# Balaji-Kesavan/DistributedDataparallel

Hardware: AMD Instinct MI355X
Metric: images/sec (whole node) ResNet-50 DDP at 1/2/4/8 MI355X; scaling efficiency (higher is better)
Workload: dtype bf16; 1 GPU; model=resnet50, global_batch=256, per_gpu_batch=256, micro_batch=256, image_size=224, parallelism=dp1, impl=xddp, backend=rccl, norm=xddp, optimizer=SGD(lr=0.1, momentum=0.9, wd=0.0001) fp32 master weights, recipe=default, miopen_implicit_gemm=default, optimizer_schedule=after backward, channels_last=True, comm_dtype=none, gradient_as_bucket_view=True

## Files before the change

distributeddataparallel_amd/csrc/kernels/conv_gemm.hip:

```cpp
#include <c10/hip/HIPStream.h>
#include <torch/extension.h>

#include "common.h"
#include "kernels/dev_utils.h"

namespace xddp {
namespace kernels {

namespace {

typedef __bf16 bf16x8 __attribute__((ext_vector_type(8)));
using dev::f32x4;
using dev::u32x4;

constexpr int kBK = 64;
constexpr bool NTSTORE = true;

__device__ __forceinline__ int swz(int row, int chunk) { return row * 128 + 16 * (chunk ^ ((row >> 1) & 7)); }

__device__ __forceinline__ void lds_barrier() { asm volatile("s_waitcnt lgkmcnt(0)\n\ts_barrier" ::: "memory"); }

__device__ __forceinline__ float bf16_round(float v) { return __uint_as_float(dev::pack_bf16x2(v, 0.f) << 16); }

typedef short v4s __attribute__((ext_vector_type(4)));

__device__ __forceinline__ v4s lds_tr16(const uint8_t* p) {
  return __builtin_amdgcn_ds_read_tr16_b64_v4i16((__attribute__((address_space(3))) v4s*)(p));
}

struct EpiBN {
  const uint16_t* add;
  const uint16_t* y;
  const uint8_t* bits;
  const float* mean;
  float* part;
  const float* ss;
  int add_h, add_w;
};

struct ProOut {
  uint16_t* out;
  uint8_t* bits;
  const float* rss;
  int64_t* nbt1;
  int64_t* nbt2;
};

struct RowMap {
  int OH, OW, IH, IW, stride;
  template <bool STRIDED>
  __device__ __forceinline__ int64_t in_row(int m) const {
    if (!STRIDED) return m;
    const int hw = OH * OW;
    const int n = m / hw, r = m - n * hw;
    const int oh = r / OW, ow = r - oh * OW;
    return ((int64_t)n * IH + oh * stride) * IW + (int64_t)ow * stride;
  }
};

template <int BM, int BN, int WM, int WN, int PRO, bool STATS, bool STRIDED, bool BT = false, bool EPI = false,
          int OCC = 4>
__global__ __launch_bounds__(64 * WM * WN, OCC) void conv1x1_gemm_kernel(
    const uint16_t* __restrict__ X, const uint16_t* __restrict__ Wt, uint16_t* __restrict__ Y, int64_t M, int N,
    int K, RowMap rm, const float* __restrict__ pro_ss, float* __restrict__ part, int mtiles, int ntiles,
    int groups, const uint16_t* __restrict__ X2, EpiBN epi, ProOut po) {
  static_assert(PRO < 4 || (!STRIDED && !BT && !EPI), "the block-output prologue is a stride-1 forward");
  constexpr int NT = 64 * WM * WN, RSTEP = NT / 8;
  constexpr int AR = BM / RSTEP, BR = BN / RSTEP;
  constexpr int WTM = BM / WM, WTN = BN / WN;
  constexpr int TM = WTM / 16, TN = WTN / 16;
  constexpr int SBT = BN * 2 + 32;
  constexpr int ABYTES = BM * 128, BBYTES = BT ? 64 * SBT : BN * 128, BUF = ABYTES + BBYTES;
  extern __shared__ __attribute__((aligned(16))) uint8_t smem[];

  const int tid = threadIdx.x, lane = tid & 63, wid = tid >> 6, wm = wid / WN, wn = wid % WN;
  const int wg = dev::xcd_remap(blockIdx.x, gridDim.x);
  const int nt = wg % ntiles, g = wg / ntiles;
  if (g >= groups) return;
  const int n0 = nt * BN;
  const int lc = tid & 7, lr = tid >> 3;
  const int nk = K / kBK;

  constexpr int CPR = BN / 8;
  static_assert(NT % CPR == 0, "readout mapping needs a fixed chunk column per thread");
  const int cc = tid % CPR;
  float st_s[8], st_ss[8];
#pragma unroll
  for (int e = 0; e < 8; ++e) st_s[e] = st_ss[e] = 0.f;
  constexpr int SPR = BN / 2, SRS = NT / SPR;
  static_assert(SPR <= 64 && 64 % SPR == 0 && BM % SRS == 0, "stats pass mapping");
  const int sp = tid % SPR;
  float sn = 0.f, sk[2] = {0.f, 0.f}, ssum[2] = {0.f, 0.f}, ssq[2] = {0.f, 0.f};

  const uint16_t* wrow[BR];
  constexpr int BCH = BN / 8;
  static_assert(!BT || 64 * BCH == NT * BR, "BT staging must cover the B tile exactly");
#pragma unroll
  for (int i = 0; i < BR; ++i) {
    if (BT) {
      const int q = tid + NT * i, row = q / BCH, c = q % BCH;
      wrow[i] = Wt + (int64_t)row * N + n0 + c * 8;
    } else {
      wrow[i] = Wt + (int64_t)(n0 + lr + RSTEP * i) * K + lc * 8;
    }
  }

  u32x4 sa[AR], sb[BR], sa2[PRO >= 2 ? AR : 1];
  float* pro_lds = reinterpret_cast<float*>(smem + 2 * BUF);
  constexpr int NCOEF = PRO == 3 ? 5 : PRO == 2 ? 3 : PRO == 5 ? 4 : PRO ? 2 : 0;
// ... 437 lines not shown
  const float dm = n > 0.f ? s1 / n : 0.f;
  const float mean = K + dm;
  const float m2 = fmaxf(s2 - s1 * dm, 0.f);
  const float Mf = M > 0 ? (float)M : n;
  const float var = Mf > 0.f ? fmaxf(m2 / Mf, 0.f) : 0.f;
  const float inv = rsqrtf(var + eps);
  mean_out[c] = mean;
  invstd_out[c] = inv;
  scale[c] = gm * inv;
  shift[c] = bb - mean * gm * inv;
  if (running_mean) {
    const float unbiased = Mf > 1.f ? var * Mf / (Mf - 1.f) : var;
    dev::Elem<W, float>::st(running_mean, c, (1.f - mom) * rm + mom * mean);
    dev::Elem<W, float>::st(running_var, c, (1.f - mom) * rv + mom * unbiased);
  }
}



template <int TN, int TK, bool STRIDED, int PRO>
__global__ __launch_bounds__(256, 2) void conv1x1_wgrad_kernel(const uint16_t* __restrict__ dY,
                                                                const uint16_t* __restrict__ X,
                                                                float* __restrict__ ws, int M, int N, int K,
                                                                RowMap rm, int ntiles, int ktiles, int mchunk,
                                                                const uint16_t* __restrict__ Y2,
                                                                const float* __restrict__ coef) {
  constexpr int BM = 64;
  constexpr int SA = TN * 2 + 32, SB = TK * 2 + 32;
  constexpr int ABYTES = BM * SA, BUF = ABYTES + BM * SB;
  constexpr int CA = TN / 8, CB = TK / 8;
  constexpr int LA = BM * CA / 256, LB = BM * CB / 256;
  constexpr int WTN = TN / 2, WTK = TK / 2, FN = WTN / 16, FK = WTK / 16;
  extern __shared__ __attribute__((aligned(16))) uint8_t smem[];

  const int tid = threadIdx.x, lane = tid & 63, wid = tid >> 6, wn = wid >> 1, wk = wid & 1;
  const int tiles = ntiles * ktiles;
  const int bid = dev::xcd_remap(blockIdx.x, gridDim.x);
  const int sidx = bid / tiles, tile = bid % tiles;
  const int n0 = (tile % ntiles) * TN, k0 = (tile / ntiles) * TK;
  const int m_begin = sidx * mchunk, m_end = min(M, m_begin + mchunk);

  u32x4 sa[2][LA], sb[2][LB], sa2[2][PRO ? LA : 1];
  float pa[8], pb[8], pc[8], pms[8], pmt[8];
  if (PRO) {
    const int c = tid % CA;
    dev::Vec8<float>::ld(coef + n0 + c * 8, pa);
    dev::Vec8<float>::ld(coef + N + n0 + c * 8, pb);
    dev::Vec8<float>::ld(coef + 2 * N + n0 + c * 8, pc);
    if (PRO == 3) {
      dev::Vec8<float>::ld(coef + 3 * N + n0 + c * 8, pms);
      dev::Vec8<float>::ld(coef + 4 * N + n0 + c * 8, pmt);
    }
  }
  auto load = [&](int slot, int m) {
#pragma unroll
    for (int i = 0; i < LA; ++i) {
      const int q = tid + 256 * i, row = q / CA, c = q - (q / CA) * CA;
      const int64_t off = (int64_t)min(m + row, M - 1) * N + n0 + c * 8;
      sa[slot][i] = *reinterpret_cast<const u32x4*>(dY + off);
      if (PRO) sa2[slot][i] = *reinterpret_cast<const u32x4*>(Y2 + off);
    }
#pragma unroll
    for (int i = 0; i < LB; ++i) {
      const int q = tid + 256 * i, row = q / CB, c = q - (q / CB) * CB;
      sb[slot][i] = *reinterpret_cast<const u32x4*>(X + rm.in_row<STRIDED>(min(m + row, M - 1)) * K + k0 + c * 8);
    }
  };
  auto store = [&](int buf, int slot, int m) {
    uint8_t* A = smem + buf * BUF;
    uint8_t* B = A + ABYTES;
#pragma unroll
    for (int i = 0; i < LA; ++i) {
      const int q = tid + 256 * i, row = q / CA, c = q - (q / CA) * CA;
      u32x4 t = sa[slot][i];
      if (PRO) {
#pragma unroll
        for (int h = 0; h < 4; ++h) {
          float g0 = __uint_as_float(sa[slot][i][h] << 16), g1 = __uint_as_float(sa[slot][i][h] & 0xffff0000u);
          const float x0 = __uint_as_float(sa2[slot][i][h] << 16), x1 = __uint_as_float(sa2[slot][i][h] & 0xffff0000u);
          if (PRO == 3) {
            g0 = fmaf(x0, pms[2 * h], pmt[2 * h]) > 0.f ? g0 : 0.f;
            g1 = fmaf(x1, pms[2 * h + 1], pmt[2 * h + 1]) > 0.f ? g1 : 0.f;
          }
          t[h] = dev::pack_bf16x2(fmaf(pa[2 * h], g0, fmaf(pb[2 * h], x0, pc[2 * h])),
                                  fmaf(pa[2 * h + 1], g1, fmaf(pb[2 * h + 1], x1, pc[2 * h + 1])));
        }
      }
      *reinterpret_cast<u32x4*>(A + row * SA + c * 16) = m + row < m_end ? t : u32x4{0, 0, 0, 0};
    }
#pragma unroll
    for (int i = 0; i < LB; ++i) {
      const int q = tid + 256 * i, row = q / CB, c = q - (q / CB) * CB;
      *reinterpret_cast<u32x4*>(B + row * SB + c * 16) = m + row < m_end ? sb[slot][i] : u32x4{0, 0, 0, 0};
    }
  };

  f32x4 acc[FN][FK];
#pragma unroll
  for (int i = 0; i < FN; ++i)
#pragma unroll
    for (int j = 0; j < FK; ++j) acc[i][j] = f32x4{0.f, 0.f, 0.f, 0.f};

  const int g = lane >> 4, q4 = (lane & 15) >> 2, p4 = lane & 3;
  auto compute = [&](int cur) {
    const uint8_t* A = smem + cur * BUF;
    const uint8_t* B = A + ABYTES;
#pragma unroll
    for (int s2 = 0; s2 < 2; ++s2) {
      const int r0 = s2 * 32 + 8 * g + q4;
      bf16x8 a[FN], b[FK];
#pragma unroll
      for (int i = 0; i < FN; ++i) {
        const int col = wn * WTN + i * 16 + 4 * p4;
        const v4s lo = lds_tr16(A + r0 * SA + col * 2), hi = lds_tr16(A + (r0 + 4) * SA + col * 2);
        const v4s v8[2] = {lo, hi};
        a[i] = __builtin_bit_cast(bf16x8, v8);
      }
#pragma unroll
      for (int j = 0; j < FK; ++j) {
        const int col = wk * WTK + j * 16 + 4 * p4;
        const v4s lo = lds_tr16(B + r0 * SB + col * 2), hi = lds_tr16(B + (r0 + 4) * SB + col * 2);
        const v4s v8[2] = {lo, hi};
        b[j] = __builtin_bit_cast(bf16x8, v8);
      }
#pragma unroll
      for (int i = 0; i < FN; ++i)
#pragma unroll
        for (int j = 0; j < FK; ++j) acc[i][j] = __builtin_amdgcn_mfma_f32_16x16x32_bf16(a[i], b[j], acc[i][j], 0, 0, 0);
    }
  };
  if (m_begin < m_end) {
    load(0, m_begin);
    load(1, m_begin + BM);
    store(0, 0, m_begin);
    lds_barrier();
    for (int m = m_begin; m < m_end; m += 2 * BM) {
      load(0, m + 2 * BM);
      compute(0);
      store(1, 1, m + BM);
      lds_barrier();
      if (m + BM >= m_end) break;
      load(1, m + 3 * BM);
      compute(1);
      store(0, 0, m + 2 * BM);
      lds_barrier();
    }
    asm volatile("s_waitcnt vmcnt(0)" ::: "memory");
  }
  float* out = ws + (int64_t)sidx * N * K;
#pragma unroll
  for (int i = 0; i < FN; ++i)
#pragma unroll
    for (int j = 0; j < FK; ++j)
#pragma unroll
      for (int r = 0; r < 4; ++r) {
        const int n = n0 + wn * WTN + i * 16 + (lane >> 4) * 4 + r;
        const int k = k0 + wk * WTK + j * 16 + (lane & 15);
        out[(int64_t)n * K + k] = acc[i][j][r];
      }
}

template <int N, int K, int PRO>
__global__ __launch_bounds__(256, 1) void conv1x1_bwd_fused_kernel(
    const uint16_t* __restrict__ G, const uint16_t* __restrict__ Y2, const float* __restrict__ coef,
    const uint16_t* __restrict__ X, const uint16_t* __restrict__ Wg, uint16_t* __restrict__ dX, float* __restrict__ ws,
    int M, int mchunk) {
  constexpr int BM = 64;
  constexpr int SA = N * 2 + 32, SB = K * 2 + 32, SW = K * 2 + 32;
  constexpr int ABYTES = BM * SA, BUF = ABYTES + BM * SB;
  constexpr int CA = N / 8, CB = K / 8;
  constexpr int LA = BM * CA / 256, LB = BM * CB / 256;
  constexpr int WTN = N / 2, WTK = K / 2, FN = WTN / 16, FK = WTK / 16;
  constexpr int KW = K / 4, KF = KW / 16;
  static_assert(256 % CA == 0 && LA >= 1 && LB >= 1 && KF >= 1, "fused 1x1 backward tile");
  extern __shared__ __attribute__((aligned(16))) uint8_t smem[];
  uint8_t* Wl = smem + 2 * BUF;

  const int tid = threadIdx.x, lane = tid & 63, wid = tid >> 6, wn = wid >> 1, wk = wid & 1;
  const int bid = dev::xcd_remap(blockIdx.x, gridDim.x);
  const int m_begin = bid * mchunk, m_end = min(M, m_begin + mchunk);

  for (int q = tid; q < N * CB; q += 256) {
    const int n = q / CB, c = q % CB;
    *reinterpret_cast<u32x4*>(Wl + n * SW + c * 16) = *reinterpret_cast<const u32x4*>(Wg + (int64_t)n * K + c * 8);
  }
  float pa[8], pb[8], pc[8], pms[8], pmt[8];
  {
    const int c = tid % CA;
    dev::Vec8<float>::ld(coef + c * 8, pa);
    dev::Vec8<float>::ld(coef + N + c * 8, pb);
    dev::Vec8<float>::ld(coef + 2 * N + c * 8, pc);
    if (PRO == 3) {
      dev::Vec8<float>::ld(coef + 3 * N + c * 8, pms);
      dev::Vec8<float>::ld(coef + 4 * N + c * 8, pmt);
    }
  }
  u32x4 sa[LA], sa2[LA], sb[LB];
  auto load = [&](int m) {
#pragma unroll
    for (int i = 0; i < LA; ++i) {
// ... 299 lines not shown
    epi = EpiBN{reinterpret_cast<const uint16_t*>(epi_add->data_ptr()), reinterpret_cast<const uint16_t*>(epi_y->data_ptr()),
                epi_bits->data_ptr<uint8_t>(), epi_mean->data_ptr<float>(), part.data_ptr<float>(), nullptr,
                epi_add_stride == 2 ? (int)OH : 0, epi_add_stride == 2 ? (int)OW : 0};
  else if (epi_form2)
    epi = EpiBN{nullptr, reinterpret_cast<const uint16_t*>(epi_y->data_ptr()), nullptr, epi_mean->data_ptr<float>(),
                part.data_ptr<float>(), epi_ss->data_ptr<float>(), 0, 0};
  RowMap rm{(int)OH, (int)OW, (int)IH, (int)IW, (int)stride};
  const dim3 grid(groups * ntiles);
  const size_t bbytes = w_t ? (size_t)64 * (BN * 2 + 32) : (size_t)BN * 128;
  const size_t lds = 2 * ((size_t)BM * 128 + bbytes) + (pro ? (pro == 5 ? 4 : ncoef) * K * sizeof(float) : 0) +
                     (epi_on ? 3 * (size_t)BN * sizeof(float) : 0);
  const auto* x2p = pro >= 4 ? reinterpret_cast<const uint16_t*>(pro_res->data_ptr())
                   : pro >= 2 ? reinterpret_cast<const uint16_t*>(prologue_y->data_ptr()) : nullptr;
  const ProOut po{def(pro_out) ? reinterpret_cast<uint16_t*>(pro_out->data_ptr()) : nullptr,
                  def(pro_bits) ? pro_bits->data_ptr<uint8_t>() : nullptr,
                  has_rss ? pro_res_ss->data_ptr<float>() : nullptr,
                  def(pro_nbt) ? pro_nbt->data_ptr<int64_t>() : nullptr,
                  def(pro_res_nbt) ? pro_res_nbt->data_ptr<int64_t>() : nullptr};
  const auto* xp = reinterpret_cast<const uint16_t*>(x.data_ptr());
  const auto* wp = reinterpret_cast<const uint16_t*>(wc.data_ptr());
  auto* yp = reinterpret_cast<uint16_t*>(y.data_ptr());
  const float* pss = pro ? prologue_ss->data_ptr<float>() : nullptr;
  float* pp = stats ? part.data_ptr<float>() : nullptr;
#define XDDP_LG(BN_, WM_, WN_, OCC_)                                                                            \
  launch_gemm<128, BN_, WM_, WN_, OCC_>(pro, stats, w_t, grid, lds, stream, xp, wp, yp, M, (int)N, (int)K, rm, pss, pp, \
                                        mtiles, ntiles, groups, x2p, epi, po)
  if (pro >= 4) {
    auto go = [&](auto kern) {
      ensure_dyn_lds((const void*)kern, lds);
      hipLaunchKernelGGL(kern, grid, dim3(512), lds, stream, xp, wp, yp, M, (int)N, (int)K, rm, pss, pp, mtiles, ntiles,
                         groups, x2p, epi, po);
    };
#define XDDP_P45(BM_, BN_, WM_, WN_)                                                                     \
    if (pro == 5) { if (stats) go(conv1x1_gemm_kernel<BM_, BN_, WM_, WN_, 5, true, false, false, false, 4>);    \
                    else go(conv1x1_gemm_kernel<BM_, BN_, WM_, WN_, 5, false, false, false, false, 4>); }   \
    else { if (stats) go(conv1x1_gemm_kernel<BM_, BN_, WM_, WN_, 4, true, false, false, false, 4>);             \
           else go(conv1x1_gemm_kernel<BM_, BN_, WM_, WN_, 4, false, false, false, false, 4>); }
    if (BN == 128) { XDDP_P45(64, 128, 2, 4) } else { XDDP_P45(128, 64, 8, 1) }
#undef XDDP_P45
    XDDP_HIP_CHECK(hipGetLastError());
  } else if (bm64) {
    auto kern = pro == 2 ? conv1x1_gemm_kernel<64, 128, 2, 4, 2, false, false, true, true, 4>
                         : conv1x1_gemm_kernel<64, 128, 2, 4, 0, false, false, true, true, 4>;
    hipLaunchKernelGGL(kern, grid, dim3(512), lds, stream, xp, wp, yp, M, (int)N, (int)K, rm, pss, pp, mtiles, ntiles,
                       groups, x2p, epi, po);
    XDDP_HIP_CHECK(hipGetLastError());
  } else if (BN == 128) { if (kocc == 2) XDDP_LG(128, 4, 2, 2); else XDDP_LG(128, 4, 2, 4); }
  else { if (kocc == 2) XDDP_LG(64, 8, 1, 2); else XDDP_LG(64, 8, 1, 4); }
#undef XDDP_LG
  return {y, part};
}


at::Tensor conv1x1_wgrad(const at::Tensor& dy, const at::Tensor& x, int64_t stride, const at::Tensor& w_like,
                         const c10::optional<at::Tensor>& prologue_y, const c10::optional<at::Tensor>& coef) {
  const auto wdtype = w_like.scalar_type();
  const bool has_y2 = prologue_y.has_value() && prologue_y->defined();
  const int pro = has_y2 ? (coef.has_value() && coef->defined() && coef->numel() == 5 * dy.size(1) ? 3 : 2) : 0;
  TORCH_CHECK(dy.is_cuda() && x.is_cuda() && dy.scalar_type() == at::kBFloat16 && x.scalar_type() == at::kBFloat16,
              "conv1x1_wgrad: bf16 GPU tensors expected");
  TORCH_CHECK(dy.dim() == 4 && x.dim() == 4 && dy.is_contiguous(at::MemoryFormat::ChannelsLast) &&
                  x.is_contiguous(at::MemoryFormat::ChannelsLast), "conv1x1_wgrad: channels_last 4-D tensors expected");
  const int64_t B = x.size(0), K = x.size(1), IH = x.size(2), IW = x.size(3), N = dy.size(1);
  const int64_t OH = (IH - 1) / stride + 1, OW = (IW - 1) / stride + 1;
  TORCH_CHECK(dy.size(0) == B && dy.size(2) == OH && dy.size(3) == OW, "conv1x1_wgrad: dy/x shape mismatch");
  TORCH_CHECK(N % 64 == 0 && K % 64 == 0, "conv1x1_wgrad: channel counts must be multiples of 64");
  const int64_t M = B * OH * OW;
  TORCH_CHECK(M > 0 && M < (int64_t(1) << 31), "conv1x1_wgrad: bad M");
  if (pro)
    TORCH_CHECK(prologue_y->sizes() == dy.sizes() && prologue_y->scalar_type() == at::kBFloat16 &&
                    prologue_y->is_contiguous(at::MemoryFormat::ChannelsLast) && stride == 1 && coef.has_value() &&
                    coef->defined() && coef->scalar_type() == at::kFloat && coef->numel() == (pro == 3 ? 5 : 3) * N &&
                    coef->is_contiguous(),
                "conv1x1_wgrad: prologue_y must match dy (bf16 channels_last, stride 1) with float coef [3|5, N]");
  const auto* y2p = pro ? reinterpret_cast<const uint16_t*>(prologue_y->data_ptr()) : nullptr;
  const float* cfp = pro ? coef->data_ptr<float>() : nullptr;
  const int TN = N % 128 == 0 ? 128 : 64, TK = K % 128 == 0 ? 128 : 64;
  const int ntiles = (int)(N / TN), ktiles = (int)(K / TK), tiles = ntiles * ktiles;
  const int64_t steps = (M + 63) / 64;
  int S = (int)std::max<int64_t>(1, std::min<int64_t>(steps, (int64_t)num_cus() * 2 / tiles));
  const int64_t mchunk = ((steps + S - 1) / S) * 64;
  S = (int)((M + mchunk - 1) / mchunk);
  auto ws = at::empty({S, N, K}, dy.options().dtype(at::kFloat));
  auto dw = at::empty({N, K, 1, 1}, dy.options().dtype(wdtype));
  auto stream = c10::hip::getCurrentHIPStream(dy.device().index()).stream();
  RowMap rm{(int)OH, (int)OW, (int)IH, (int)IW, (int)stride};
  const size_t lds = 2 * (size_t)64 * ((TN * 2 + 32) + (TK * 2 + 32));
  auto go = [&](auto kern) {
    ensure_dyn_lds((const void*)kern, lds);
    hipLaunchKernelGGL(kern, dim3(S * tiles), dim3(256), lds, stream,
                       reinterpret_cast<const uint16_t*>(dy.data_ptr()), reinterpret_cast<const uint16_t*>(x.data_ptr()),
                       ws.data_ptr<float>(), (int)M, (int)N, (int)K, rm, ntiles, ktiles, (int)mchunk, y2p, cfp);
    XDDP_HIP_CHECK(hipGetLastError());
  };
  const bool strided = stride > 1;
#define XDDP_W(A, Bk) \
  if (pro == 3) go(conv1x1_wgrad_kernel<A, Bk, false, 3>);                                         \
  else if (pro == 2) go(conv1x1_wgrad_kernel<A, Bk, false, 2>);                                    \
  else if (strided) go(conv1x1_wgrad_kernel<A, Bk, true, 0>); else go(conv1x1_wgrad_kernel<A, Bk, false, 0>)
  if (TN == 128 && TK == 128) { XDDP_W(128, 128); }
  else if (TN == 128) { XDDP_W(128, 64); }
  else if (TK == 128) { XDDP_W(64, 128); }
  else { XDDP_W(64, 64); }
#undef XDDP_W
  const int64_t nk = N * K;
  const int grid = (int)((nk / 4 + 63) / 64);
  auto red = [&](auto tag) {
    using W = decltype(tag);
    hipLaunchKernelGGL((wgrad_reduce_kernel<W>), dim3(grid), dim3(512), 0, stream, ws.data_ptr<float>(), S, nk,
                       reinterpret_cast<W*>(dw.data_ptr()));
    XDDP_HIP_CHECK(hipGetLastError());
  };
  switch (wdtype) {
    case at::kBFloat16: red(dev::bf16_t{}); break;
    case at::kFloat: red(float{}); break;
    case at::kHalf: red(dev::f16_t{}); break;
    default: TORCH_CHECK(false, "conv1x1_wgrad: unsupported weight dtype");
  }
  return dw;
}

bool conv1x1_bwd_fused_supported(int64_t N, int64_t K) { return (N == 256 && K == 64) || (N == 64 && K == 256); }

std::vector<at::Tensor> conv1x1_bwd_fused(const at::Tensor& g, const at::Tensor& y2, const at::Tensor& coef,
                                          const at::Tensor& x, const at::Tensor& w) {
  TORCH_CHECK(g.is_cuda() && g.scalar_type() == at::kBFloat16 && g.dim() == 4 &&
                  g.is_contiguous(at::MemoryFormat::ChannelsLast) && y2.sizes() == g.sizes() &&
                  y2.scalar_type() == at::kBFloat16 && y2.is_contiguous(at::MemoryFormat::ChannelsLast),
              "conv1x1_bwd_fused: g, y2 must be matching bf16 channels_last tensors");
  const int64_t B = x.size(0), K = x.size(1), H = x.size(2), Wd = x.size(3), N = g.size(1);
  TORCH_CHECK(x.scalar_type() == at::kBFloat16 && x.is_contiguous(at::MemoryFormat::ChannelsLast) &&
                  g.size(0) == B && g.size(2) == H && g.size(3) == Wd,
              "conv1x1_bwd_fused: x must be bf16 channels_last with g's batch and spatial size (stride 1)");
  TORCH_CHECK(conv1x1_bwd_fused_supported(N, K), "conv1x1_bwd_fused: unsupported (N, K)");
  TORCH_CHECK(w.scalar_type() == at::kBFloat16 && w.numel() == N * K && w.size(0) == N && w.is_contiguous(),
              "conv1x1_bwd_fused: w must be contiguous bf16 [N, K, 1, 1]");
  const int pro = coef.numel() == 5 * N ? 3 : 2;
  TORCH_CHECK(coef.scalar_type() == at::kFloat && coef.is_contiguous() && (coef.numel() == 3 * N || pro == 3),
              "conv1x1_bwd_fused: coef must be float [3|5, N]");
  const int64_t M = B * H * Wd;
  TORCH_CHECK(M > 0 && M < (int64_t(1) << 31), "conv1x1_bwd_fused: bad M");
  const int64_t steps = (M + 63) / 64;
  int S = (int)std::max<int64_t>(1, std::min<int64_t>(steps, (int64_t)num_cus()));
  const int64_t mchunk = ((steps + S - 1) / S) * 64;
  S = (int)((M + mchunk - 1) / mchunk);
  auto dx = at::empty({B, K, H, Wd}, x.options().memory_format(at::MemoryFormat::ChannelsLast));
  auto ws = at::empty({S, N, K}, x.options().dtype(at::kFloat));
  auto dw = at::empty({N, K, 1, 1}, w.options().memory_format(at::MemoryFormat::Contiguous));
  auto stream = c10::hip::getCurrentHIPStream(x.device().index()).stream();
  const size_t lds = 2 * (size_t)64 * ((N * 2 + 32) + (K * 2 + 32)) + (size_t)N * (K * 2 + 32);
  auto go = [&](auto kern) {
    ensure_dyn_lds((const void*)kern, lds);
    hipLaunchKernelGGL(kern, dim3(S), dim3(256), lds, stream, reinterpret_cast<const uint16_t*>(g.data_ptr()),
                       reinterpret_cast<const uint16_t*>(y2.data_ptr()), coef.data_ptr<float>(),
                       reinterpret_cast<const uint16_t*>(x.data_ptr()), reinterpret_cast<const uint16_t*>(w.data_ptr()),
                       reinterpret_cast<uint16_t*>(dx.data_ptr()), ws.data_ptr<float>(), (int)M, (int)mchunk);
    XDDP_HIP_CHECK(hipGetLastError());
  };
  if (N == 256) { if (pro == 3) go(conv1x1_bwd_fused_kernel<256, 64, 3>); else go(conv1x1_bwd_fused_kernel<256, 64, 2>); }
  else { if (pro == 3) go(conv1x1_bwd_fused_kernel<64, 256, 3>); else go(conv1x1_bwd_fused_kernel<64, 256, 2>); }
  const int64_t nk = N * K;
  hipLaunchKernelGGL((wgrad_reduce_kernel<dev::bf16_t>), dim3((unsigned)((nk / 4 + 63) / 64)), dim3(512), 0, stream,
                     ws.data_ptr<float>(), S, nk, reinterpret_cast<dev::bf16_t*>(dw.data_ptr()));
  XDDP_HIP_CHECK(hipGetLastError());
  return {dx, dw};
}


std::vector<at::Tensor> bn_stats_from_partials(const at::Tensor& part, int64_t M,
                                               const c10::optional<at::Tensor>& weight,
                                               const c10::optional<at::Tensor>& bias,
                                               const c10::optional<at::Tensor>& running_mean,
// ... 36 lines not shown
```

distributeddataparallel_amd/csrc/kernels/norm.h:

```cpp
#pragma once

#include <ATen/ATen.h>
#include <pybind11/pybind11.h>

#include <tuple>
#include <vector>

namespace xddp {
namespace kernels {

std::vector<at::Tensor> bn_forward(const at::Tensor& x, const c10::optional<at::Tensor>& weight,
                                   const c10::optional<at::Tensor>& bias, const c10::optional<at::Tensor>& running_mean,
                                   const c10::optional<at::Tensor>& running_var,
                                   const c10::optional<at::Tensor>& num_batches_tracked, bool training,
                                   double momentum, bool cumulative, double eps,
                                   const c10::optional<at::Tensor>& residual, bool relu, bool save_mask);
std::vector<at::Tensor> bn_backward(const at::Tensor& dy, const at::Tensor& x, const c10::optional<at::Tensor>& y,
                                    const c10::optional<at::Tensor>& weight, const at::Tensor& mean,
                                    const at::Tensor& invstd, const c10::optional<at::Tensor>& ss, bool relu,
                                    bool need_dres, bool need_dweight, const c10::optional<at::Tensor>& dy2,
                                    const c10::optional<at::Tensor>& mask_bits, bool coef_only);
at::Tensor bn_moments(const at::Tensor& x);
at::Tensor bn_grad_partials(const at::Tensor& dy, const at::Tensor& x, const at::Tensor& mean);
std::vector<at::Tensor> bn_apply(const at::Tensor& x, const at::Tensor& ss, const c10::optional<at::Tensor>& residual,
                                 bool relu, bool save_mask, const c10::optional<at::Tensor>& num_batches_tracked,
                                 const c10::optional<at::Tensor>& residual_ss,
                                 const c10::optional<at::Tensor>& residual_nbt, const c10::optional<at::Tensor>& out,
                                 const c10::optional<at::Tensor>& out_bits);
std::vector<at::Tensor> conv1x1_gemm(const at::Tensor& x, const at::Tensor& w, int64_t stride,
                                     const c10::optional<at::Tensor>& prologue_ss, bool stats,
                                     const c10::optional<at::Tensor>& prologue_y, bool w_t,
                                     const c10::optional<at::Tensor>& epi_add, const c10::optional<at::Tensor>& epi_y,
                                     const c10::optional<at::Tensor>& epi_bits, const c10::optional<at::Tensor>& epi_mean,
                                     const c10::optional<at::Tensor>& epi_ss, int64_t epi_add_stride,
                                     const c10::optional<at::Tensor>& pro_out, const c10::optional<at::Tensor>& pro_bits,
                                     const c10::optional<at::Tensor>& pro_res, const c10::optional<at::Tensor>& pro_res_ss,
                                     const c10::optional<at::Tensor>& pro_nbt, const c10::optional<at::Tensor>& pro_res_nbt);
std::vector<at::Tensor> bn_backward_from_partials(const at::Tensor& part, int64_t M,
                                                  const c10::optional<at::Tensor>& weight, const at::Tensor& mean,
                                                  const at::Tensor& invstd, bool need_dweight, bool fold_mean);
bool bn_tail_timeouts(int64_t device);
at::Tensor bn_backward_elem(const at::Tensor& g, const at::Tensor& x, const at::Tensor& mean, const at::Tensor& coef);
std::vector<at::Tensor> gemm_nt(const at::Tensor& a, const at::Tensor& w, const c10::optional<at::Tensor>& bias,
                                int64_t epi, const c10::optional<at::Tensor>& residual,
                                const c10::optional<at::Tensor>& out);
at::Tensor fp8_amax(const at::Tensor& x);
std::tuple<at::Tensor, c10::optional<at::Tensor>, at::Tensor> fp8_quantize(const at::Tensor& x, const at::Tensor& amax,
                                                                           int64_t fmt, bool transpose);
at::Tensor gemm_fp8_nt(const at::Tensor& a, const at::Tensor& b, const at::Tensor& scale_a, const at::Tensor& scale_b,
                       int64_t a_fmt, int64_t b_fmt, int64_t epi, const c10::optional<at::Tensor>& residual,
                       const c10::optional<at::Tensor>& out);
std::vector<at::Tensor> conv3x3_forward(const at::Tensor& x, const at::Tensor& w, int64_t stride, bool stats);
std::vector<at::Tensor> conv3x3_gemm(const at::Tensor& x, const at::Tensor& w, int64_t stride, bool stats,
                                     const uint16_t* zeros);
std::vector<at::Tensor> conv3x3_band(const at::Tensor& x, const at::Tensor& w, bool stats, int64_t rows,
                                     const uint16_t* zeros, int64_t cfg = -1);
int conv3x3_band_rows(int64_t W, int64_t H, int64_t bm);
std::vector<at::Tensor> conv3x3_band_forward(const at::Tensor& x, const at::Tensor& w, bool stats, int64_t rows,
                                             int64_t cfg);
at::Tensor conv3x3_rot_weight(const at::Tensor& w);
std::vector<at::Tensor> conv3x3_rot_weights(const std::vector<at::Tensor>& ws);
at::Tensor conv3x3_dgrad_s2(const at::Tensor& dy, const at::Tensor& w_rot, int64_t H, int64_t W);
at::Tensor conv3x3_dgrad_s2_gemm(const at::Tensor& dy, const at::Tensor& wr, int64_t XH, int64_t XW,
                                 const uint16_t* zeros);
at::Tensor conv3x3_wgrad_patch(const at::Tensor& dy, const at::Tensor& x, int64_t stride, const at::Tensor& w_like,
                               int64_t splits = -1);
at::Tensor conv1x1_wgrad(const at::Tensor& dy, const at::Tensor& x, int64_t stride, const at::Tensor& w_like,
                         const c10::optional<at::Tensor>& prologue_y, const c10::optional<at::Tensor>& coef);
bool conv1x1_bwd_fused_supported(int64_t N, int64_t K);
std::vector<at::Tensor> conv1x1_bwd_fused(const at::Tensor& g, const at::Tensor& y2, const at::Tensor& coef,
                                          const at::Tensor& x, const at::Tensor& w);
std::vector<at::Tensor> bn_stats_from_partials(const at::Tensor& part, int64_t M,
                                               const c10::optional<at::Tensor>& weight,
                                               const c10::optional<at::Tensor>& bias,
                                               const c10::optional<at::Tensor>& running_mean,
                                               const c10::optional<at::Tensor>& running_var,
                                               const c10::optional<at::Tensor>& num_batches_tracked, double momentum,
                                               bool cumulative, double eps, bool group_minor);
std::vector<at::Tensor> ln_forward(const at::Tensor& x, const c10::optional<at::Tensor>& gamma,
                                   const c10::optional<at::Tensor>& beta, double eps, bool rms,
                                   const c10::optional<at::Tensor>& add_bias);
std::vector<at::Tensor> ln_backward(const at::Tensor& dy, const at::Tensor& x, const c10::optional<at::Tensor>& gamma,
                                    const c10::optional<at::Tensor>& mean, const at::Tensor& rstd, bool rms,
                                    bool need_dgamma, bool need_dbeta, const c10::optional<at::Tensor>& res);
void colsum_partials(const at::Tensor& part, at::Tensor& out);

std::vector<at::Tensor> maxpool_forward(const at::Tensor& x, int64_t k, int64_t stride, int64_t pad);
at::Tensor global_avg_pool_backward(const at::Tensor& g, const at::Tensor& x_like);
std::vector<at::Tensor> stem_conv_forward(const at::Tensor& x, const at::Tensor& w);
at::Tensor stem_conv_wgrad(const at::Tensor& dy, const at::Tensor& x, const at::Tensor& w_like);
std::vector<at::Tensor> stem_pool_forward(const at::Tensor& x, const at::Tensor& ss);
at::Tensor stem_pool_bn_backward(const at::Tensor& dy, const c10::optional<at::Tensor>& dy2, const at::Tensor& idx,
                                 const at::Tensor& x, const at::Tensor& ss, const at::Tensor& mean,
                                 const c10::optional<at::Tensor>& coef);
at::Tensor maxpool_backward(const at::Tensor& dy, const at::Tensor& idx, const at::Tensor& x_like, int64_t k,
                            int64_t stride, int64_t pad, const c10::optional<at::Tensor>& dy2);

at::Tensor rope(const at::Tensor& x, const at::Tensor& cosv, const at::Tensor& sinv, bool backward,
                const c10::optional<at::Tensor>& positions = c10::nullopt);
at::Tensor swiglu_forward(const at::Tensor& a, const at::Tensor& b);
std::vector<at::Tensor> swiglu_backward(const at::Tensor& g, const at::Tensor& a, const at::Tensor& b);
at::Tensor gelu_forward(const at::Tensor& h);
at::Tensor transpose16(const at::Tensor& x);
std::vector<at::Tensor> bias_grad(const at::Tensor& g, const c10::optional<at::Tensor>& gelu_input,
                                  const at::Tensor& bias_like);

std::vector<at::Tensor> flash_attn_forward(const at::Tensor& q, const at::Tensor& k, const at::Tensor& v, bool causal,
                                           double scale, const c10::optional<at::Tensor>& doc_start = c10::nullopt);
std::vector<at::Tensor> flash_attn_backward(const at::Tensor& dout, const at::Tensor& q, const at::Tensor& k,
                                            const at::Tensor& v, const at::Tensor& o, const at::Tensor& lse,
                                            bool causal, double scale, const c10::optional<at::Tensor>& dq_out,
                                            const c10::optional<at::Tensor>& dk_out,
                                            const c10::optional<at::Tensor>& dv_out,
                                            const c10::optional<at::Tensor>& bias_like,
                                            const c10::optional<at::Tensor>& doc_start = c10::nullopt,
                                            const c10::optional<at::Tensor>& doc_end = c10::nullopt);

void bind_norm_kernels(pybind11::module_& m);

std::vector<at::Tensor> cross_entropy_forward(const at::Tensor& logits, const at::Tensor& target, int64_t ignore_index,
                                              const at::Tensor& bad);
// ... 6 lines not shown
```

distributeddataparallel_amd/csrc/kernels/norm_bind.cpp:

```cpp
#include <torch/extension.h>

#include "kernels/norm.h"

namespace py = pybind11;

namespace xddp {
namespace kernels {

void bind_norm_kernels(py::module_& m) {
  m.def("bn_forward", &bn_forward, py::arg("x"), py::arg("weight"), py::arg("bias"), py::arg("running_mean"),
        py::arg("running_var"), py::arg("num_batches_tracked"), py::arg("training"), py::arg("momentum"),
        py::arg("cumulative"), py::arg("eps"), py::arg("residual"), py::arg("relu"), py::arg("save_mask") = false);
  m.def("bn_backward", &bn_backward, py::arg("dy"), py::arg("x"), py::arg("y"), py::arg("weight"), py::arg("mean"),
        py::arg("invstd"), py::arg("scale_shift"), py::arg("relu"), py::arg("need_dres"), py::arg("need_dweight"),
        py::arg("dy2") = py::none(), py::arg("mask_bits") = py::none(), py::arg("coef_only") = false);
  m.def("bn_apply", &bn_apply, py::arg("x"), py::arg("scale_shift"), py::arg("residual"), py::arg("relu"),
        py::arg("save_mask"), py::arg("num_batches_tracked"), py::arg("residual_ss") = py::none(),
        py::arg("residual_nbt") = py::none(), py::arg("out") = py::none(), py::arg("out_bits") = py::none());
  m.def("conv1x1_gemm", &conv1x1_gemm, py::arg("x"), py::arg("w"), py::arg("stride"), py::arg("prologue_ss"),
        py::arg("stats"), py::arg("prologue_y") = py::none(), py::arg("w_t") = false, py::arg("epi_add") = py::none(),
        py::arg("epi_y") = py::none(), py::arg("epi_bits") = py::none(), py::arg("epi_mean") = py::none(),
        py::arg("epi_ss") = py::none(), py::arg("epi_add_stride") = 1, py::arg("pro_out") = py::none(),
        py::arg("pro_bits") = py::none(), py::arg("pro_res") = py::none(), py::arg("pro_res_ss") = py::none(),
        py::arg("pro_nbt") = py::none(), py::arg("pro_res_nbt") = py::none());
  m.def("bn_backward_from_partials", &bn_backward_from_partials, py::arg("partials"), py::arg("M"), py::arg("weight"),
        py::arg("mean"), py::arg("invstd"), py::arg("need_dweight"), py::arg("fold_mean") = true);
  m.def("bn_tail_timeouts", &bn_tail_timeouts, py::arg("device"),
        "whether a folded BN finalize hit its spin bound since the last call (clears the flag; synchronizes)");
  m.def("bn_backward_elem", &bn_backward_elem, py::arg("g"), py::arg("x"), py::arg("mean"), py::arg("coef"));
  m.def("bn_moments", &bn_moments, py::arg("x"));
  m.def("cross_entropy_forward", &cross_entropy_forward, py::arg("logits"), py::arg("target"),
        py::arg("ignore_index"), py::arg("bad"));
  m.def("cross_entropy_backward", &cross_entropy_backward, py::arg("logits"), py::arg("target"), py::arg("lse"),
        py::arg("gscale"), py::arg("ignore_index") = -100);
  m.def("bn_grad_partials", &bn_grad_partials, py::arg("dy"), py::arg("x"), py::arg("mean"));
  m.def("conv3x3_forward", &conv3x3_forward, py::arg("x"), py::arg("w"), py::arg("stride"), py::arg("stats"));
  m.def("conv3x3_rot_weight", &conv3x3_rot_weight, py::arg("w"));
  m.def("conv3x3_rot_weights", &conv3x3_rot_weights, py::arg("ws"));
  m.def("conv3x3_band_forward", &conv3x3_band_forward, py::arg("x"), py::arg("w"), py::arg("stats"),
        py::arg("rows") = 0, py::arg("cfg") = -1);
  m.def("conv3x3_dgrad_s2", &conv3x3_dgrad_s2, py::arg("dy"), py::arg("w_rot"), py::arg("H"), py::arg("W"));
  m.def("conv3x3_wgrad_patch", &conv3x3_wgrad_patch, py::arg("dy"), py::arg("x"), py::arg("stride"), py::arg("w_like"),
        py::arg("splits") = -1);
  m.def("conv1x1_bwd_fused_supported", &conv1x1_bwd_fused_supported, py::arg("N"), py::arg("K"));
  m.def("conv1x1_bwd_fused", &conv1x1_bwd_fused, py::arg("g"), py::arg("y2"), py::arg("coef"), py::arg("x"),
        py::arg("w"));
  m.def("conv1x1_wgrad", &conv1x1_wgrad, py::arg("dy"), py::arg("x"), py::arg("stride"), py::arg("w_like"),
        py::arg("prologue_y") = py::none(), py::arg("coef") = py::none());
  m.def("bn_stats_from_partials", &bn_stats_from_partials, py::arg("partials"), py::arg("M"), py::arg("weight"),
        py::arg("bias"), py::arg("running_mean"), py::arg("running_var"), py::arg("num_batches_tracked"),
        py::arg("momentum"), py::arg("cumulative"), py::arg("eps"), py::arg("group_minor") = false);
  m.def("gemm_nt", &gemm_nt, py::arg("a"), py::arg("w"), py::arg("bias") = py::none(), py::arg("epi") = 0,
        py::arg("residual") = py::none(), py::arg("out") = py::none(),
        "y = a @ w.T (bf16, MFMA LDS-DMA GEMM) with epilogue 0 none | 1 +bias | 2 +bias->GELU | 3 +residual | "
        "4 GELU backward (residual = h): {(a @ w.T) * gelu'(h), column sums} | 5 BatchNorm statistics: "
        "{y, partials [3, N, mtiles] group-minor}");
  m.def("fp8_amax", &fp8_amax, py::arg("x"), "max |x| of a bf16 tensor -> float32[1] (device, no host sync)");
  m.def("fp8_quantize", &fp8_quantize, py::arg("x"), py::arg("amax"), py::arg("fmt"), py::arg("transpose"),
        "x [R, C] bf16 -> (q [R, C] uint8, qT [C, R] uint8 or None, scale float32[1]); fmt 0 e4m3 | 1 e5m2 (OCP), "
        "q = fp8(clamp(x * scale, +-FMAX)), scale = FMAX / amax (1 for amax = 0)");
  m.def("gemm_fp8_nt", &gemm_fp8_nt, py::arg("a"), py::arg("b"), py::arg("scale_a"), py::arg("scale_b"),
        py::arg("a_fmt"), py::arg("b_fmt"), py::arg("epi") = 0, py::arg("res") = py::none(), py::arg("out") = py::none(),
        "bf16 y = (a @ b.T) / (scale_a * scale_b) on FP8 bytes (block-scaled MFMA, unit block scales); epi 1: + res "
        "(res may be out)");
  m.def("flash_attn_forward", &flash_attn_forward, py::arg("q"), py::arg("k"), py::arg("v"), py::arg("causal"),
        py::arg("scale"), py::arg("doc_start") = py::none());
  m.def("flash_attn_backward", &flash_attn_backward, py::arg("dout"), py::arg("q"), py::arg("k"), py::arg("v"),
        py::arg("o"), py::arg("lse"), py::arg("causal"), py::arg("scale"), py::arg("dq_out") = py::none(),
        py::arg("dk_out") = py::none(), py::arg("dv_out") = py::none(), py::arg("bias_like") = py::none(),
        py::arg("doc_start") = py::none(), py::arg("doc_end") = py::none());
  m.def("rope", &rope, py::arg("x"), py::arg("cos"), py::arg("sin"), py::arg("backward") = false,
        py::arg("positions") = py::none());
  m.def("swiglu_forward", &swiglu_forward, py::arg("a"), py::arg("b"));
  m.def("swiglu_backward", &swiglu_backward, py::arg("grad"), py::arg("a"), py::arg("b"));
  m.def("stem_conv_forward", &stem_conv_forward, py::arg("x"), py::arg("w"));
  m.def("stem_conv_wgrad", &stem_conv_wgrad, py::arg("dy"), py::arg("x"), py::arg("w_like"));
  m.def("stem_pool_forward", &stem_pool_forward, py::arg("x"), py::arg("scale_shift"));
  m.def("stem_pool_bn_backward", &stem_pool_bn_backward, py::arg("dy"), py::arg("dy2"), py::arg("idx"), py::arg("x"),
        py::arg("scale_shift"), py::arg("mean"), py::arg("coef") = py::none());
  m.def("maxpool_forward", &maxpool_forward, py::arg("x"), py::arg("kernel"), py::arg("stride"), py::arg("pad"));
  m.def("global_avg_pool_backward", &global_avg_pool_backward, py::arg("g"), py::arg("x_like"));
  m.def("maxpool_backward", &maxpool_backward, py::arg("dy"), py::arg("idx"), py::arg("x_like"), py::arg("kernel"),
        py::arg("stride"), py::arg("pad"), py::arg("dy2") = py::none());
  m.def("ln_forward", &ln_forward, py::arg("x"), py::arg("gamma"), py::arg("beta"), py::arg("eps"), py::arg("rms"),
        py::arg("add_bias") = py::none());
  m.def("ln_backward", &ln_backward, py::arg("dy"), py::arg("x"), py::arg("gamma"), py::arg("mean"), py::arg("rstd"),
        py::arg("rms"), py::arg("need_dgamma"), py::arg("need_dbeta"), py::arg("res") = py::none());
  m.def("gelu_forward", &gelu_forward, py::arg("h"));
  m.def("transpose16", &transpose16, py::arg("x"));
  m.def("bias_grad", &bias_grad, py::arg("grad"), py::arg("gelu_input") = py::none(), py::arg("bias_like"));
}

}
}
```

Measured before the change: 13770 images/s.

## Add wide-tile 512-thread wgrad kernel with split-M reduction and incremental strided row walk

Adds a conv1x1 weight-gradient kernel that uses 512 threads and 128x256 or 256x128 output tiles. Two wave halves split the M dimension and their partial sums are reduced through LDS. The host picks it automatically for large N*K layers without a prologue, and launches about one block per CU instead of two, which raises operand reuse per block. Separately, the strided row-address computation is replaced in both kernels by an incremental walker that avoids per-load integer divisions. The cost is more registers and LDS per block, lower occupancy, and the extra cross-half reduction step.

Result: no change. 13850 images/s (median of 6 runs) (+0.6%).

```diff
diff --git a/distributeddataparallel_amd/csrc/kernels/conv_gemm.hip b/distributeddataparallel_amd/csrc/kernels/conv_gemm.hip
--- a/distributeddataparallel_amd/csrc/kernels/conv_gemm.hip
+++ b/distributeddataparallel_amd/csrc/kernels/conv_gemm.hip
@@ -55,6 +55,37 @@
     const int n = m / hw, r = m - n * hw;
     const int oh = r / OW, ow = r - oh * OW;
     return ((int64_t)n * IH + oh * stride) * IW + (int64_t)ow * stride;
+  }
+};
+
+struct RowStep {
+  int d_oh, d_ow;
+  int64_t d_in, c_ow, c_oh;
+  __device__ __forceinline__ RowStep(const RowMap& rm, int D) {
+    const int hw = rm.OH * rm.OW, qi = D / hw, r = D - qi * hw;
+    d_oh = r / rm.OW;
+    d_ow = r - d_oh * rm.OW;
+    d_in = ((int64_t)qi * rm.IH + d_oh * rm.stride) * rm.IW + d_ow * rm.stride;
+    c_ow = (int64_t)rm.stride * (rm.IW - rm.OW);
+    c_oh = (int64_t)rm.IW * (rm.IH - rm.OH * rm.stride);
+  }
+};
+struct RowWalk {
+  int oh, ow;
+  int64_t in;
+  __device__ __forceinline__ void init(const RowMap& rm, int m) {
+    const int hw = rm.OH * rm.OW;
+    const int n = m / hw, r = m - n * hw;
+    oh = r / rm.OW;
+    ow = r - oh * rm.OW;
+    in = ((int64_t)n * rm.IH + oh * rm.stride) * rm.IW + (int64_t)ow * rm.stride;
+  }
+  __device__ __forceinline__ void advance(const RowMap& rm, const RowStep& st) {
+    in += st.d_in;
+    ow += st.d_ow;
+    if (ow >= rm.OW) { ow -= rm.OW; oh += 1; in += st.c_ow; }
+    oh += st.d_oh;
+    if (oh >= rm.OH) { oh -= rm.OH; in += st.c_oh; }
   }
 };
 
@@ -598,6 +629,13 @@
       dev::Vec8<float>::ld(coef + 4 * N + n0 + c * 8, pmt);
     }
   }
+  const RowStep rstep(rm, BM);
+  RowWalk rw[STRIDED ? LB : 1];
+  const int64_t in_last = rm.in_row<STRIDED>(M - 1);
+  if (STRIDED) {
+#pragma unroll
+    for (int i = 0; i < LB; ++i) rw[i].init(rm, m_begin + (tid + 256 * i) / CB);
+  }
   auto load = [&](int slot, int m) {
 #pragma unroll
     for (int i = 0; i < LA; ++i) {
@@ -609,7 +647,12 @@
 #pragma unroll
     for (int i = 0; i < LB; ++i) {
       const int q = tid + 256 * i, row = q / CB, c = q - (q / CB) * CB;
-      sb[slot][i] = *reinterpret_cast<const u32x4*>(X + rm.in_row<STRIDED>(min(m + row, M - 1)) * K + k0 + c * 8);
+      int64_t in = min(m + row, M - 1);
+      if (STRIDED) {
+        in = min(rw[i].in, in_last);
+        rw[i].advance(rm, rstep);
+      }
+      sb[slot][i] = *reinterpret_cast<const u32x4*>(X + in * K + k0 + c * 8);
     }
   };
   auto store = [&](int buf, int slot, int m) {
@@ -692,6 +735,175 @@
       lds_barrier();
     }
     asm volatile("s_waitcnt vmcnt(0)" ::: "memory");
+  }
+  float* out = ws + (int64_t)sidx * N * K;
+#pragma unroll
+  for (int i = 0; i < FN; ++i)
+#pragma unroll
+    for (int j = 0; j < FK; ++j)
+#pragma unroll
+      for (int r = 0; r < 4; ++r) {
+        const int n = n0 + wn * WTN + i * 16 + (lane >> 4) * 4 + r;
+        const int k = k0 + wk * WTK + j * 16 + (lane & 15);
+        out[(int64_t)n * K + k] = acc[i][j][r];
+      }
+}
+
+template <int TN, int TK, bool STRIDED, int PRO>
+__global__ __launch_bounds__(512, 1) void conv1x1_wgrad_wide_kernel(
+    const uint16_t* __restrict__ dY, const uint16_t* __restrict__ X, float* __restrict__ ws, int M, int N, int K,
+    RowMap rm, int ntiles, int ktiles, int mchunk, const uint16_t* __restrict__ Y2,
+    const float* __restrict__ coef) {
+  constexpr int NT = 512, BM = 64;
+  constexpr int SA = TN * 2 + 32, SB = TK * 2 + 32;
+  constexpr int ABYTES = BM * SA, BUF = ABYTES + BM * SB;
+  constexpr int CA = TN / 8, CB = TK / 8;
+  constexpr int LA = BM * CA / NT, LB = BM * CB / NT;
+  constexpr int WTN = TN / 2, WTK = TK / 2, FN = WTN / 16, FK = WTK / 16;
+  static_assert(LA >= 1 && LB >= 1 && NT % CA == 0 && NT % CB == 0, "staging layout");
+  extern __shared__ __attribute__((aligned(16))) uint8_t smem[];
+
+  const int tid = threadIdx.x, lane = tid & 63, wid = tid >> 6;
+  const int wh = wid >> 2, wn = (wid >> 1) & 1, wk = wid & 1;
+  const int tiles = ntiles * ktiles;
+  const int bid = dev::xcd_remap(blockIdx.x, gridDim.x);
+  const int sidx = bid / tiles, tile = bid % tiles;
+  const int n0 = (tile % ntiles) * TN, k0 = (tile / ntiles) * TK;
+  const int m_begin = sidx * mchunk, m_end = min(M, m_begin + mchunk);
+
+  u32x4 sa[2][LA], sb[2][LB], sa2[2][PRO ? LA : 1];
+  float pa[8], pb[8], pc[8], pms[8], pmt[8];
+  if (PRO) {
+    const int c = tid % CA;
+    dev::Vec8<float>::ld(coef + n0 + c * 8, pa);
+    dev::Vec8<float>::ld(coef + N + n0 + c * 8, pb);
+    dev::Vec8<float>::ld(coef + 2 * N + n0 + c * 8, pc);
+    if (PRO == 3) {
+      dev::Vec8<float>::ld(coef + 3 * N + n0 + c * 8, pms);
+      dev::Vec8<float>::ld(coef + 4 * N + n0 + c * 8, pmt);
+    }
+  }
+  const RowStep rstep(rm, BM);
+  RowWalk rw[STRIDED ? LB : 1];
+  const int64_t in_last = rm.in_row<STRIDED>(M - 1);
+  if (STRIDED) {
+#pragma unroll
+    for (int i = 0; i < LB; ++i) rw[i].init(rm, m_begin + (tid + NT * i) / CB);
+  }
+  auto load = [&](int slot, int m) {
+#pragma unroll
+    for (int i = 0; i < LA; ++i) {
+      const int q = tid + NT * i, row = q / CA, c = q - (q / CA) * CA;
+      const int64_t off = (int64_t)min(m + row, M - 1) * N + n0 + c * 8;
+      sa[slot][i] = *reinterpret_cast<const u32x4*>(dY + off);
+      if (PRO) sa2[slot][i] = *reinterpret_cast<const u32x4*>(Y2 + off);
+    }
+#pragma unroll
+    for (int i = 0; i < LB; ++i) {
+      const int q = tid + NT * i, row = q / CB, c = q - (q / CB) * CB;
+      int64_t in = min(m + row, M - 1);
+      if (STRIDED) {
+        in = min(rw[i].in, in_last);
+        rw[i].advance(rm, rstep);
+      }
+      sb[slot][i] = *reinterpret_cast<const u32x4*>(X + in * K + k0 + c * 8);
+    }
+  };
+  auto store = [&](int buf, int slot, int m) {
+    uint8_t* A = smem + buf * BUF;
+    uint8_t* B = A + ABYTES;
+#pragma unroll
+    for (int i = 0; i < LA; ++i) {
+      const int q = tid + NT * i, row = q / CA, c = q - (q / CA) * CA;
+      u32x4 t = sa[slot][i];
+      if (PRO) {
+#pragma unroll
+        for (int h = 0; h < 4; ++h) {
+          float g0 = __uint_as_float(sa[slot][i][h] << 16), g1 = __uint_as_float(sa[slot][i][h] & 0xffff0000u);
+          const float x0 = __uint_as_float(sa2[slot][i][h] << 16), x1 = __uint_as_float(sa2[slot][i][h] & 0xffff0000u);
+          if (PRO == 3) {
+            g0 = fmaf(x0, pms[2 * h], pmt[2 * h]) > 0.f ? g0 : 0.f;
+            g1 = fmaf(x1, pms[2 * h + 1], pmt[2 * h + 1]) > 0.f ? g1 : 0.f;
+          }
+          t[h] = dev::pack_bf16x2(fmaf(pa[2 * h], g0, fmaf(pb[2 * h], x0, pc[2 * h])),
+                                  fmaf(pa[2 * h + 1], g1, fmaf(pb[2 * h + 1], x1, pc[2 * h + 1])));
+        }
+      }
+      *reinterpret_cast<u32x4*>(A + row * SA + c * 16) = m + row < m_end ? t : u32x4{0, 0, 0, 0};
+    }
+#pragma unroll
+    for (int i = 0; i < LB; ++i) {
+      const int q = tid + NT * i, row = q / CB, c = q - (q / CB) * CB;
+      *reinterpret_cast<u32x4*>(B + row * SB + c * 16) = m + row < m_end ? sb[slot][i] : u32x4{0, 0, 0, 0};
+    }
+  };
+
+  f32x4 acc[FN][FK];
+#pragma unroll
+  for (int i = 0; i < FN; ++i)
+#pragma unroll
+    for (int j = 0; j < FK; ++j) acc[i][j] = f32x4{0.f, 0.f, 0.f, 0.f};
+
+  const int g = lane >> 4, q4 = (lane & 15) >> 2, p4 = lane & 3;
+  auto compute = [&](int cur) {
+    const uint8_t* A = smem + cur * BUF;
+    const uint8_t* B = A + ABYTES;
+    {
+      const int r0 = wh * 32 + 8 * g + q4;
+      bf16x8 a[FN], b[FK];
+#pragma unroll
+      for (int i = 0; i < FN; ++i) {
+        const int col = wn * WTN + i * 16 + 4 * p4;
+        const v4s lo = lds_tr16(A + r0 * SA + col * 2), hi = lds_tr16(A + (r0 + 4) * SA + col * 2);
+        const v4s v8[2] = {lo, hi};
+        a[i] = __builtin_bit_cast(bf16x8, v8);
+      }
+#pragma unroll
+      for (int j = 0; j < FK; ++j) {
+        const int col = wk * WTK + j * 16 + 4 * p4;
+        const v4s lo = lds_tr16(B + r0 * SB + col * 2), hi = lds_tr16(B + (r0 + 4) * SB + col * 2);
+        const v4s v8[2] = {lo, hi};
+        b[j] = __builtin_bit_cast(bf16x8, v8);
+      }
+#pragma unroll
+      for (int i = 0; i < FN; ++i)
+#pragma unroll
+        for (int j = 0; j < FK; ++j) acc[i][j] = __builtin_amdgcn_mfma_f32_16x16x32_bf16(a[i], b[j], acc[i][j], 0, 0, 0);
+    }
+  };
+  if (m_begin < m_end) {
+    load(0, m_begin);
+    load(1, m_begin + BM);
+    store(0, 0, m_begin);
+    lds_barrier();
+    for (int m = m_begin; m < m_end; m += 2 * BM) {
+      load(0, m + 2 * BM);
+      compute(0);
+      store(1, 1, m + BM);
+      lds_barrier();
+      if (m + BM >= m_end) break;
+      load(1, m + 3 * BM);
+      compute(1);
+      store(0, 0, m + 2 * BM);
+      lds_barrier();
+    }
+    asm volatile("s_waitcnt vmcnt(0)" ::: "memory");
+  }
+  {
+    f32x4* red = reinterpret_cast<f32x4*>(smem) + (wid & 3) * (FN * FK * 64) + lane;
+    __syncthreads();
+    if (wh == 1) {
+#pragma unroll
+      for (int i = 0; i < FN; ++i)
+#pragma unroll
+        for (int j = 0; j < FK; ++j) red[(i * FK + j) * 64] = acc[i][j];
+    }
+    __syncthreads();
+    if (wh == 1) return;
+#pragma unroll
+    for (int i = 0; i < FN; ++i)
+#pragma unroll
+      for (int j = 0; j < FK; ++j) acc[i][j] += red[(i * FK + j) * 64];
   }
   float* out = ws + (int64_t)sidx * N * K;
 #pragma unroll
@@ -1097,8 +1309,11 @@
 }
 
 
-at::Tensor conv1x1_wgrad(const at::Tensor& dy, const at::Tensor& x, int64_t stride, const at::Tensor& w_like,
-                         const c10::optional<at::Tensor>& prologue_y, const c10::optional<at::Tensor>& coef) {
+bool wgrad_wide_wins(int64_t N, int64_t K, int pro) { return pro == 0 && N * K >= 128 * 512; }
+
+at::Tensor conv1x1_wgrad_variant(const at::Tensor& dy, const at::Tensor& x, int64_t stride, const at::Tensor& w_like,
+                                 const c10::optional<at::Tensor>& prologue_y, const c10::optional<at::Tensor>& coef,
+                                 int64_t variant) {
   const auto wdtype = w_like.scalar_type();
   const bool has_y2 = prologue_y.has_value() && prologue_y->defined();
   const int pro = has_y2 ? (coef.has_value() && coef->defined() && coef->numel() == 5 * dy.size(1) ? 3 : 2) : 0;
@@ -1120,33 +1335,46 @@
                 "conv1x1_wgrad: prologue_y must match dy (bf16 channels_last, stride 1) with float coef [3|5, N]");
   const auto* y2p = pro ? reinterpret_cast<const uint16_t*>(prologue_y->data_ptr()) : nullptr;
   const float* cfp = pro ? coef->data_ptr<float>() : nullptr;
-  const int TN = N % 128 == 0 ? 128 : 64, TK = K % 128 == 0 ? 128 : 64;
+  const bool strided = stride > 1;
+  const bool wide_ok = N % 128 == 0 && K % 128 == 0 && (N % 256 == 0 || K % 256 == 0);
+  TORCH_CHECK(variant >= -1 && variant <= 1 && (variant != 1 || wide_ok),
+              "conv1x1_wgrad: the wide kernel needs N, K multiples of 128 and one of them of 256");
+  const bool wide = variant < 0 ? wide_ok && wgrad_wide_wins(N, K, pro) : variant == 1;
+  int TN = N % 128 == 0 ? 128 : 64, TK = K % 128 == 0 ? 128 : 64;
+  if (wide) {
+    const bool k256 = K % 256 == 0 && !(strided && N % 256 == 0);
+    TN = k256 ? 128 : 256;
+    TK = k256 ? 256 : 128;
+  }
   const int ntiles = (int)(N / TN), ktiles = (int)(K / TK), tiles = ntiles * ktiles;
   const int64_t steps = (M + 63) / 64;
-  int S = (int)std::max<int64_t>(1, std::min<int64_t>(steps, (int64_t)num_cus() * 2 / tiles));
+  int S = (int)std::max<int64_t>(
+      1, std::min<int64_t>(steps, (int64_t)num_cus() * (wide ? 1 : 2) / tiles));
   const int64_t mchunk = ((steps + S - 1) / S) * 64;
   S = (int)((M + mchunk - 1) / mchunk);
   auto ws = at::empty({S, N, K}, dy.options().dtype(at::kFloat));
   auto dw = at::empty({N, K, 1, 1}, dy.options().dtype(wdtype));
   auto stream = c10::hip::getCurrentHIPStream(dy.device().index()).stream();
   RowMap rm{(int)OH, (int)OW, (int)IH, (int)IW, (int)stride};
-  const size_t lds = 2 * (size_t)64 * ((TN * 2 + 32) + (TK * 2 + 32));
+  size_t lds = 2 * (size_t)64 * ((TN * 2 + 32) + (TK * 2 + 32));
+  if (wide) lds = std::max(lds, (size_t)TN * TK * 4);
   auto go = [&](auto kern) {
     ensure_dyn_lds((const void*)kern, lds);
-    hipLaunchKernelGGL(kern, dim3(S * tiles), dim3(256), lds, stream,
+    hipLaunchKernelGGL(kern, dim3(S * tiles), dim3(wide ? 512 : 256), lds, stream,
                        reinterpret_cast<const uint16_t*>(dy.data_ptr()), reinterpret_cast<const uint16_t*>(x.data_ptr()),
                        ws.data_ptr<float>(), (int)M, (int)N, (int)K, rm, ntiles, ktiles, (int)mchunk, y2p, cfp);
     XDDP_HIP_CHECK(hipGetLastError());
   };
-  const bool strided = stride > 1;
-#define XDDP_W(A, Bk) \
-  if (pro == 3) go(conv1x1_wgrad_kernel<A, Bk, false, 3>);                                         \
-  else if (pro == 2) go(conv1x1_wgrad_kernel<A, Bk, false, 2>);                                    \
-  else if (strided) go(conv1x1_wgrad_kernel<A, Bk, true, 0>); else go(conv1x1_wgrad_kernel<A, Bk, false, 0>)
-  if (TN == 128 && TK == 128) { XDDP_W(128, 128); }
-  else if (TN == 128) { XDDP_W(128, 64); }
-  else if (TK == 128) { XDDP_W(64, 128); }
-  else { XDDP_W(64, 64); }
+#define XDDP_W(KERN, ...) \
+  if (pro == 3) go(KERN<__VA_ARGS__, false, 3>);                                         \
+  else if (pro == 2) go(KERN<__VA_ARGS__, false, 2>);                                    \
+  else if (strided) go(KERN<__VA_ARGS__, true, 0>); else go(KERN<__VA_ARGS__, false, 0>)
+  if (wide && TN == 128) { XDDP_W(conv1x1_wgrad_wide_kernel, 128, 256); }
+  else if (wide) { XDDP_W(conv1x1_wgrad_wide_kernel, 256, 128); }
+  else if (TN == 128 && TK == 128) { XDDP_W(conv1x1_wgrad_kernel, 128, 128); }
+  else if (TN == 128) { XDDP_W(conv1x1_wgrad_kernel, 128, 64); }
+  else if (TK == 128) { XDDP_W(conv1x1_wgrad_kernel, 64, 128); }
+  else { XDDP_W(conv1x1_wgrad_kernel, 64, 64); }
 #undef XDDP_W
   const int64_t nk = N * K;
   const int grid = (int)((nk / 4 + 63) / 64);
@@ -1163,6 +1391,11 @@
     default: TORCH_CHECK(false, "conv1x1_wgrad: unsupported weight dtype");
   }
   return dw;
+}
+
+at::Tensor conv1x1_wgrad(const at::Tensor& dy, const at::Tensor& x, int64_t stride, const at::Tensor& w_like,
+                         const c10::optional<at::Tensor>& prologue_y, const c10::optional<at::Tensor>& coef) {
+  return conv1x1_wgrad_variant(dy, x, stride, w_like, prologue_y, coef, -1);
 }
 
 bool conv1x1_bwd_fused_supported(int64_t N, int64_t K) { return (N == 256 && K == 64) || (N == 64 && K == 256); }
diff --git a/distributeddataparallel_amd/csrc/kernels/norm.h b/distributeddataparallel_amd/csrc/kernels/norm.h
--- a/distributeddataparallel_amd/csrc/kernels/norm.h
+++ b/distributeddataparallel_amd/csrc/kernels/norm.h
@@ -67,6 +67,9 @@
                                int64_t splits = -1);
 at::Tensor conv1x1_wgrad(const at::Tensor& dy, const at::Tensor& x, int64_t stride, const at::Tensor& w_like,
                          const c10::optional<at::Tensor>& prologue_y, const c10::optional<at::Tensor>& coef);
+at::Tensor conv1x1_wgrad_variant(const at::Tensor& dy, const at::Tensor& x, int64_t stride, const at::Tensor& w_like,
+                                 const c10::optional<at::Tensor>& prologue_y, const c10::optional<at::Tensor>& coef,
+                                 int64_t variant);
 bool conv1x1_bwd_fused_supported(int64_t N, int64_t K);
 std::vector<at::Tensor> conv1x1_bwd_fused(const at::Tensor& g, const at::Tensor& y2, const at::Tensor& coef,
                                           const at::Tensor& x, const at::Tensor& w);
diff --git a/distributeddataparallel_amd/csrc/kernels/norm_bind.cpp b/distributeddataparallel_amd/csrc/kernels/norm_bind.cpp
--- a/distributeddataparallel_amd/csrc/kernels/norm_bind.cpp
+++ b/distributeddataparallel_amd/csrc/kernels/norm_bind.cpp
@@ -47,6 +47,8 @@
         py::arg("w"));
   m.def("conv1x1_wgrad", &conv1x1_wgrad, py::arg("dy"), py::arg("x"), py::arg("stride"), py::arg("w_like"),
         py::arg("prologue_y") = py::none(), py::arg("coef") = py::none());
+  m.def("conv1x1_wgrad_variant", &conv1x1_wgrad_variant, py::arg("dy"), py::arg("x"), py::arg("stride"),
+        py::arg("w_like"), py::arg("prologue_y") = py::none(), py::arg("coef") = py::none(), py::arg("variant") = -1);
   m.def("bn_stats_from_partials", &bn_stats_from_partials, py::arg("partials"), py::arg("M"), py::arg("weight"),
         py::arg("bias"), py::arg("running_mean"), py::arg("running_var"), py::arg("num_batches_tracked"),
         py::arg("momentum"), py::arg("cumulative"), py::arg("eps"), py::arg("group_minor") = false);
```
